# leonardsiegert/PULPo

Measured on AMD Instinct MI355X. Metric: volume-pairs/sec fwd+bwd, 160^3 fp32, higher is better.
Workload: dtype f32

## Files before the change

### include/pulpo_hip.h

```cpp
#ifndef PULPO_HIP_H
#define PULPO_HIP_H

#include <stddef.h>
#include <stdint.h>

#ifdef __cplusplus
extern "C" {
#endif

#define PULPO_ABI_VERSION 8
int pulpo_abi_version(void);
const char* pulpo_last_error(void);

size_t pulpo_conv3d_k3_packed_floats(int K, int N);
int pulpo_conv3d_k3_pack_weight(const float* w , float* wp, int Cin, int Cout, int dgrad, void* stream);
int pulpo_conv3d_k3_stat_tiles(int B, int D, int H, int W);
int pulpo_conv3d_k3_tile_config(int K, int N);
size_t pulpo_conv3d_k3_fwd_scratch_floats(int B, int D, int H, int W, int K, int N);
int pulpo_conv3d_k3_fwd(const float* in, int64_t in_bs, int64_t in_ps, int64_t in_cs, const float* wp, const float* bias, float* out,
                        int64_t out_bs, int64_t out_ps, int64_t out_cs, float* stats, float* scratch , int B,
                        int D, int H, int W, int K, int N, void* stream);
int pulpo_conv3d_k3_fwd_bn_lrelu(const float* in, int64_t in_bs, int64_t in_ps, int64_t in_cs, const float* wp, const float* bias,
                                 const float* coef, float slope, float* out, int64_t out_bs, int64_t out_ps, int64_t out_cs, float* scratch, int B,
                                 int D, int H, int W, int K, int N, void* stream);
// ... 231 lines not shown
int pulpo_bn_lrelu_apply_t(const void* y, int y_dt, int64_t yps, void* z, int z_dt, int64_t zps, const float* coef, int64_t npix, int C, float slope,
                           void* stream);
int pulpo_bn_lrelu_apply_pool2_t(const void* y, int y_dt, int64_t yps, void* z , int z_dt, int64_t zps,
                                 void* pooled , int64_t pps,
                                 const float* coef, int B, int D, int H, int W, int C, float slope, void* stream);
int pulpo_bn_lrelu_bwd_reduce_t(const void* dz, int dz_dt, int64_t dzps, const void* y, int y_dt, int64_t yps, const float* coef, int64_t npix, int C,
                                float slope, float* partial, void* stream);
int pulpo_bn_lrelu_bwd_apply_t(const void* dz, int dz_dt, int64_t dzps, const void* y, int y_dt, int64_t yps, const float* coef, const double* totd,
                               void* dy , int64_t dyps, int64_t npix, int C, float slope, float* partial2, void* stream);
int pulpo_avgpool2_bwd_bnred_t(const void* gout, int64_t gops, const void* add, int64_t aps, void* gin, int64_t gips, int g_dt ,
                               const void* y, int y_dt, int64_t yps, const float* coef, float slope, float* partial, int B, int D, int H, int W,
                               int C, void* stream);
int pulpo_heads_fwd_t(const void* h, int h_dt, int64_t ps, const float* Wt, const float* bias, const float* eps, float* o0, float* o1, float* o2,
                      int nout, int B, int64_t V, int C, void* stream);
int pulpo_heads_bwd_t(const void* h, int h_dt, int64_t ps, const float* Wt, const float* g0, const float* g1, const float* g2, const float* eps,
                      const float* sigma, void* dh , int64_t dps, float* partial, int nout, int B, int64_t V, int C, void* stream);
int pulpo_avgpool2_fwd_t(const void* in, int64_t ips, void* out, int64_t ops, int dt, int B, int D, int H, int W, int C, void* stream);
int pulpo_avgpool2_bwd_t(const void* gout, int64_t gops, const void* add , int64_t aps, void* gin, int64_t gips, int dt, int B, int D,
                         int H, int W, int C, void* stream);
int pulpo_feedback_up2_fwd_t(const float* const* srcs , const int* chans , int nsrc, void* out,
                             int dt, int64_t ops, int B, int Di, int Hi, int Wi, void* stream);
int pulpo_feedback_up2_bwd_t(const void* gout, int dt, int64_t gops, float* const* gsrcs , const int* chans,
                             int nsrc, int B, int Di, int Hi, int Wi, void* stream);

int pulpo_conv3d_k3_wgrad_bn_rows(int B, int D, int H, int W, int Cout);
int pulpo_conv3d_k3_wgrad_bn(const float* in, int64_t in_bs, int64_t in_ps, int64_t in_cs, const void* dz, int dz_dt, int64_t dz_bs, int64_t dz_ps,
                             const float* y, int64_t y_bs, int64_t y_ps, const float* coef, const double* totd, float slope, float* dw,
                             int accumulate, float* scratch, float* part2, int B, int D, int H, int W, int Cin, int Cout, void* stream);

int pulpo_bn_lrelu_bwd_apply_pooled_t(const void* gout, int64_t gops, const void* add , int64_t aps, int g_dt, const void* y, int y_dt,
                                      int64_t yps, const float* coef, const double* totd, void* dy , int64_t dyps, float slope,
                                      float* partial2, int B, int D, int H, int W, int C, void* stream);

int pulpo_bn_lrelu_apply_kb(const float* y, int64_t yps, float* z, int64_t zps, int64_t zkb, const float* coef, int64_t npix, int C, float slope, void* stream);
int pulpo_bn_lrelu_bwd_apply_kb_t(const void* dz, int dz_dt, int64_t dzps, int64_t dzkb, const float* y, int64_t yps, const float* coef, const double* totd,
                                  float* dy, int64_t dyps, int64_t dykb, int64_t npix, int C, float slope, float* partial2, void* stream);
int pulpo_conv3d_k3_wgrad_bn_kb(const float* in, int64_t in_bs, int64_t in_ps, int64_t in_cs, const float* dz, int64_t dz_bs, int64_t dz_ps, int64_t dz_kb,
                                const float* y, int64_t y_bs, int64_t y_ps, const float* coef, const double* totd, float slope, float* dw, int accumulate,
                                float* scratch, float* part2, int B, int D, int H, int W, int Cin, int Cout, void* stream);
int pulpo_bn_lrelu_bwd_apply_pooled_kb_t(const void* gout, int64_t gops, const void* add , int64_t aps, int g_dt, const float* y, int64_t yps,
                                         const float* coef, const double* totd, float* dy, int64_t dyps, int64_t dykb, float slope, float* partial2,
                                         int B, int D, int H, int W, int C, void* stream);
int pulpo_conv3d_k3_fwd_wino3_kb(const float* in, int64_t in_bs, int64_t in_ps, int64_t in_kb, const float* wp, const float* bias, const float* coef,
                                 float slope, float* out, int64_t out_bs, int64_t out_ps, int64_t out_kb, float* stats, int B, int D, int H, int W, int K,
                                 int N, void* stream);
int pulpo_conv3d_k3_dgrad_wino3_bnred_kb(const float* in, int64_t in_bs, int64_t in_ps, int64_t in_kb, const float* wp, float* out, int64_t out_bs,
                                         int64_t out_ps, int64_t out_kb, const float* bn_y, int64_t bn_y_bs, int64_t bn_y_ps, const float* bn_coef, float slope,
                                         float* part, int B, int D, int H, int W, int K, int N, void* stream);
int pulpo_conv3d_k3_wgrad_kb(const float* in, int64_t in_bs, int64_t in_ps, int64_t in_kb, const float* dy, int64_t dy_bs, int64_t dy_ps, int64_t dy_kb,
                             float* dw, int accumulate, float* scratch, float* slabs , int nslab, int B, int D, int H, int W, int Cin, int Cout,
                             void* stream);

int pulpo_conv3d_k3_wgrad_det_slabs(int Cin, int Cout);
int pulpo_conv3d_k3_wgrad_det(const float* in, int64_t in_bs, int64_t in_ps, int64_t in_cs, const float* dy, int64_t dy_bs, int64_t dy_ps,
                              int64_t dy_cs, float* dw, int accumulate, float* scratch, float* slabs, int nslab, int B, int D, int H, int W,
                              int Cin, int Cout, void* stream);
int pulpo_conv3d_k3_wgrad_bf16_det_t(const void* in, int64_t in_bs, int64_t in_ps, int64_t in_cs, const void* dy, int64_t dy_bs, int64_t dy_ps,
                                     int64_t dy_cs, int dt, float* dw, int accumulate, float* scratch, float* slabs, int nslab, int B, int D,
                                     int H, int W, int Cin, int Cout, void* stream);
int pulpo_resize_trilinear_scaled_bwd_det(const float* gout, float* gin, int64_t nplanes, int Di, int Hi, int Wi, int Do, int Ho, int Wo,
                                          float scale_d, float scale_h, float scale_w, float mult, void* stream);
size_t pulpo_warp3d_bwd_det_ws_bytes(int B, int C, int Di, int Hi, int Wi);
int pulpo_warp3d_bwd_det(const float* df, const float* img, const float* gout, float* gdf , float* gimg ,
                         void* ws , int B, int C, int Dg, int Hg, int Wg, int Di, int Hi, int Wi, void* stream);
size_t pulpo_vecint_bwd_det_ws_bytes(int B, int D, int H, int W, int nsteps);
int pulpo_vecint_bwd_det(const float* work, const float* gout, float* gin, void* ws , int B, int D, int H, int W,
// ... 30 lines not shown
```

### pulpo_amd/csrc/norm_act.hip

```cpp
#include "act_io.h"
#include "head_bn.h"

namespace {

__global__ __launch_bounds__(1024) void colsum_kernel(const float* __restrict__ partials, int nrow, int ncol, float* __restrict__ out,
                                                        float scale, int accumulate) {
    __shared__ double red[32][33];
    const int cx = threadIdx.x, ry = threadIdx.y;
    const int c = blockIdx.x * 32 + cx;
    double s = 0.0;
    if (c < ncol)
        for (int r = ry; r < nrow; r += 32) s += (double)partials[(long)r * ncol + c];
    red[ry][cx] = s;
    __syncthreads();
    if (ry == 0 && c < ncol) {
        double t = 0.0;
#pragma unroll
        for (int k = 0; k < 32; ++k) t += red[k][cx];
        const float r = (float)(t * (double)scale);
        out[c] = accumulate ? out[c] + r : r;
    }
}

constexpr int CS_RY = 8;
// ... 86 lines not shown
    coef[2 * C + c] = sc;
    coef[3 * C + c] = beta[c] - rm[c] * sc;
    double* cd = reinterpret_cast<double*>(coef + 4 * C);
    cd[c] = (double)rm[c];
    cd[C + c] = 1.0 / sqrt((double)rv[c] + (double)eps);
}

template <int VEC>
struct Vec {
    static __device__ __forceinline__ void ld(const float* p, float (&v)[VEC]) { pulpo::ldv<VEC>(p, v); }
    static __device__ __forceinline__ void st(float* p, const float (&v)[VEC]) { pulpo::stv<VEC>(p, v); }
};

template <int VEC, typename TY = float, typename TZ = float>
__global__ __launch_bounds__(256) void bn_lrelu_apply_kernel(const TY* __restrict__ y, long yps, TZ* __restrict__ z, long zps,
                                                               const float* __restrict__ coef, long npix, int C, float slope, long zkb = 8) {
    const int CV = C / VEC;
    const long total = npix * CV;
    const float* scale = coef + 2 * C;
    const float* shift = coef + 3 * C;
    for (long e = blockIdx.x * (long)blockDim.x + threadIdx.x; e < total; e += (long)gridDim.x * blockDim.x) {
        const long p = e / CV;
        const int c = (int)(e - p * CV) * VEC;
        float v[VEC], sc[VEC], sh[VEC];
        pulpo::ldv<VEC>(y + p * yps + c, v);
        Vec<VEC>::ld(scale + c, sc);
        Vec<VEC>::ld(shift + c, sh);
#pragma unroll
        for (int k = 0; k < VEC; ++k) v[k] = pulpo::bn_lrelu(v[k], sc[k], sh[k], slope);
        pulpo::stv<VEC>(z + (long)(c >> 3) * zkb + p * zps + (c & 7), v);
    }
}

template <typename TY = float, typename TZ = float>
__global__ __launch_bounds__(256) void bn_lrelu_apply_pool2_kernel(const TY* __restrict__ y, long yps, TZ* __restrict__ z, long zps,
                                                                     TZ* __restrict__ pooled, long pps, const float* __restrict__ coef, int B,
                                                                     int D, int H, int W, int Do, int Ho, int Wo, int C, float slope) {
    const int CV = C / 4;
    const long total = (long)B * Do * Ho * Wo * CV;
    const float* scale = coef + 2 * C;
    const float* shift = coef + 3 * C;
    for (long e = blockIdx.x * (long)blockDim.x + threadIdx.x; e < total; e += (long)gridDim.x * blockDim.x) {
        const int c = (int)(e % CV) * 4;
        long p = e / CV;
        const int ox = (int)(p % Wo); p /= Wo;
        const int oy = (int)(p % Ho); p /= Ho;
        const int oz = (int)(p % Do);
        const int b = (int)(p / Do);
        const int z1 = min(2 * oz + 2, D), y1 = min(2 * oy + 2, H), x1 = min(2 * ox + 2, W);
        float sc[4], sh[4], acc[4] = {0.f, 0.f, 0.f, 0.f};
        Vec<4>::ld(scale + c, sc);
        Vec<4>::ld(shift + c, sh);
        for (int zz = 2 * oz; zz < z1; ++zz)
            for (int yy = 2 * oy; yy < y1; ++yy)
                for (int xx = 2 * ox; xx < x1; ++xx) {
                    const long vox = (((long)b * D + zz) * H + yy) * W + xx;
                    float v[4];
                    pulpo::ldv<4>(y + vox * yps + c, v);
#pragma unroll
                    for (int k = 0; k < 4; ++k) {
                        v[k] = pulpo::as_stored<TZ>(pulpo::bn_lrelu(v[k], sc[k], sh[k], slope));
                        acc[k] += v[k];
                    }
                    if (z != nullptr) pulpo::stv<4>(z + vox * zps + c, v);
                }
        const float inv = 1.f / (float)((z1 - 2 * oz) * (y1 - 2 * oy) * (x1 - 2 * ox));
#pragma unroll
        for (int k = 0; k < 4; ++k) acc[k] *= inv;
        pulpo::stv<4>(pooled + ((((long)b * Do + oz) * Ho + oy) * Wo + ox) * pps + c, acc);
    }
}

template <typename TG>
struct PoolGrad {
    const TG* gpool; long gpps;
    const TG* add; long aps;
    TG* dzout; long dzops;
    int D, H, W, Do, Ho, Wo;
};

template <int VEC, bool POOL = false, typename TG = float, typename TY = float>
__global__ __launch_bounds__(256) void bn_lrelu_bwd_reduce_kernel(const TG* __restrict__ dz, long dzps, const TY* __restrict__ y,
                                                                    long yps, const float* __restrict__ coef, long npix, int C,
                                                                    float slope, float* __restrict__ partial, PoolGrad<TG> pg = PoolGrad<TG>{}) {
    extern __shared__ float red[];
    const int CV = C / VEC, RB = blockDim.x / CV;
    const int col = threadIdx.x % CV, row = threadIdx.x / CV;
    const int c = col * VEC;
    float s0[VEC], s1[VEC];
#pragma unroll
    for (int k = 0; k < VEC; ++k) s0[k] = s1[k] = 0.f;
    if (row < RB) {
        float sc[VEC], sh[VEC], m32[VEC];
        Vec<VEC>::ld(coef + 2 * C + c, sc);
        Vec<VEC>::ld(coef + 3 * C + c, sh);
        Vec<VEC>::ld(coef + c, m32);
        for (long p = (long)blockIdx.x * RB + row; p < npix; p += (long)gridDim.x * RB) {
            float g[VEC], v[VEC];
            if constexpr (POOL) {
                long q = p;
                const int x_ = (int)(q % pg.W); q /= pg.W;
                const int y_ = (int)(q % pg.H); q /= pg.H;
// ... 244 lines not shown
                                   void* stream) {
    return pulpo_bn_lrelu_apply_t(y, 0, yps, z, 0, zps, coef, npix, C, slope, stream);
}

PULPO_API int pulpo_bn_lrelu_apply_kb(const float* y, int64_t yps, float* z, int64_t zps, int64_t zkb, const float* coef, int64_t npix, int C, float slope,
                                      void* stream) {
    PULPO_REQUIRE(y && z && coef && npix > 0 && C > 0 && C % 8 == 0 && zps % 4 == 0 && zps >= 8 && zkb % 4 == 0 && zkb >= 8, "bn_lrelu_apply_kb: bad arguments");
    return apply_t(y, (long)yps, z, (long)zps, coef, (long)npix, C, slope, (hipStream_t)stream, (long)zkb);
}

PULPO_API int pulpo_bn_lrelu_apply_pool2_ok(int C, int64_t yps, int64_t zps, int64_t pps) { return C % 4 == 0 && yps % 4 == 0 && zps % 4 == 0 && pps % 4 == 0; }

PULPO_API int pulpo_bn_lrelu_apply_pool2_t(const void* y, int y_dt, int64_t yps, void* z, int z_dt, int64_t zps, void* pooled, int64_t pps,
                                           const float* coef, int B, int D, int H, int W, int C, float slope, void* stream) {
    PULPO_REQUIRE(y && pooled && coef && B > 0 && D > 0 && H > 0 && W > 0 && C > 0, "bn_lrelu_apply_pool2: bad arguments");
    PULPO_REQUIRE_DT(y_dt, "bn_lrelu_apply_pool2"); PULPO_REQUIRE_DT(z_dt, "bn_lrelu_apply_pool2");
    const int ey = y_dt ? 2 : 4, ez = z_dt ? 2 : 4;
    PULPO_REQUIRE(pulpo_bn_lrelu_apply_pool2_ok(C, yps, zps, pps) && (((uintptr_t)y) % (4 * ey)) == 0 && ((((uintptr_t)z) | ((uintptr_t)pooled)) % (4 * ez)) == 0 &&
                      (((uintptr_t)coef) & 15) == 0,
                  "bn_lrelu_apply_pool2: operands must be channels-last, aligned to four elements, C %% 4 == 0");
    const int Do = (D + 1) / 2, Ho = (H + 1) / 2, Wo = (W + 1) / 2;
    const int nb = stream_blocks((long)B * Do * Ho * Wo * (C / 4));
    PULPO_DISPATCH_DT(y_dt, TY, PULPO_DISPATCH_DT(z_dt, TZ,
        hipLaunchKernelGGL((bn_lrelu_apply_pool2_kernel<TY, TZ>), dim3(nb), dim3(256), 0, (hipStream_t)stream, (const TY*)y, (long)yps, (TZ*)z, (long)zps,
                           (TZ*)pooled, (long)pps, coef, B, D, H, W, Do, Ho, Wo, C, slope)));
    return pulpo::check_launch("bn_lrelu_apply_pool2");
}

PULPO_API int pulpo_bn_lrelu_apply_pool2(const float* y, int64_t yps, float* z, int64_t zps, float* pooled, int64_t pps, const float* coef, int B, int D,
                                         int H, int W, int C, float slope, void* stream) {
    return pulpo_bn_lrelu_apply_pool2_t(y, 0, yps, z, 0, zps, pooled, pps, coef, B, D, H, W, C, slope, stream);
}

PULPO_API int pulpo_bn_bwd_blocks(int64_t npix, int C) {
    const int vec = (C % 4 == 0) ? 4 : 1;
    const int RB = std::max(1, 256 / (C / vec));
    return (int)std::max<long>(1, std::min<long>((npix + RB * 8 - 1) / (RB * 8), 2048));
}

namespace {
inline int bwd_group(const pulpo::GroupProbe& g, bool half, int C) {
    if (half && g.ok8 && C / 8 <= 256) return 8;
    if (g.ok4) return C / 4 <= 256 ? 4 : -2;
    if (C % 4 == 0) return -1;
    return C <= 256 ? 1 : -2;
}

template <typename TG, typename TY>
int reduce_t(const TG* dz, long dzps, const TY* y, long yps, const float* coef, long npix, int C, float slope, float* partial, hipStream_t st) {
    pulpo::GroupProbe g(C);
    g.add(dz, dzps, sizeof(TG)); g.add(y, yps, sizeof(TY)); g.add(coef, 8, 4);
    const int vec = bwd_group(g, sizeof(TG) == 2 || sizeof(TY) == 2, C);
    if (vec == -1) return pulpo::fail(-1, "bn_lrelu_bwd_reduce: operands must be aligned to four elements when C %% 4 == 0");
    if (vec == -2) return pulpo::fail(-1, "bn_lrelu_bwd_reduce: too many channels (%d)", C);
    const int nblk = pulpo_bn_bwd_blocks(npix, C);
    const int RB = std::max(1, 256 / (C / vec));
    const size_t lds = (size_t)RB * 2 * C * sizeof(float);
    if (vec == 8) hipLaunchKernelGGL((bn_lrelu_bwd_reduce_kernel<8, false, TG, TY>), dim3(nblk), dim3(256), lds, st, dz, dzps, y, yps, coef, npix, C, slope, partial, PoolGrad<TG>{});
    else if (vec == 4) hipLaunchKernelGGL((bn_lrelu_bwd_reduce_kernel<4, false, TG, TY>), dim3(nblk), dim3(256), lds, st, dz, dzps, y, yps, coef, npix, C, slope, partial, PoolGrad<TG>{});
    else hipLaunchKernelGGL((bn_lrelu_bwd_reduce_kernel<1, false, TG, TY>), dim3(nblk), dim3(256), lds, st, dz, dzps, y, yps, coef, npix, C, slope, partial, PoolGrad<TG>{});
    return pulpo::check_launch("bn_lrelu_bwd_reduce");
}

template <typename TG, typename TY>
int pool_reduce_t(const TG* gout, long gops, const TG* add, long aps, TG* gin, long gips, const TY* y, long yps, const float* coef, float slope,
                  float* partial, int B, int D, int H, int W, int C, hipStream_t st) {
// ... 41 lines not shown
                                          int C, float slope, float* partial, void* stream) {
    PULPO_REQUIRE(dz && y && coef && partial && npix > 0 && C > 0, "bn_lrelu_bwd_reduce: bad arguments");
    PULPO_REQUIRE_DT(dz_dt, "bn_lrelu_bwd_reduce"); PULPO_REQUIRE_DT(y_dt, "bn_lrelu_bwd_reduce");
    PULPO_DISPATCH_DT(dz_dt, TG, PULPO_DISPATCH_DT(y_dt, TY,
        return reduce_t((const TG*)dz, (long)dzps, (const TY*)y, (long)yps, coef, (long)npix, C, slope, partial, (hipStream_t)stream)));
    return -1;
}

PULPO_API int pulpo_bn_lrelu_bwd_reduce(const float* dz, int64_t dzps, const float* y, int64_t yps, const float* coef, int64_t npix, int C,
                                        float slope, float* partial, void* stream) {
    return pulpo_bn_lrelu_bwd_reduce_t(dz, 0, dzps, y, 0, yps, coef, npix, C, slope, partial, stream);
}

PULPO_API int pulpo_avgpool2_bwd_bnred_t(const void* gout, int64_t gops, const void* add, int64_t aps, void* gin, int64_t gips, int g_dt, const void* y,
                                         int y_dt, int64_t yps, const float* coef, float slope, float* partial, int B, int D, int H, int W, int C,
                                         void* stream) {
    PULPO_REQUIRE(gout && y && coef && partial && B > 0 && D > 0 && H > 0 && W > 0 && C > 0, "avgpool2_bwd_bnred: bad arguments");
    PULPO_REQUIRE_DT(g_dt, "avgpool2_bwd_bnred"); PULPO_REQUIRE_DT(y_dt, "avgpool2_bwd_bnred");
    const int eg = g_dt ? 8 : 16, ey = y_dt ? 8 : 16;
    PULPO_REQUIRE(C % 4 == 0 && C / 4 <= 256 && gops % 4 == 0 && gips % 4 == 0 && yps % 4 == 0 && (add == nullptr || aps % 4 == 0) &&
                      ((((uintptr_t)gout) | ((uintptr_t)gin) | ((uintptr_t)add)) % eg) == 0 && (((uintptr_t)y) % ey) == 0 && (((uintptr_t)coef) & 15) == 0,
                  "avgpool2_bwd_bnred: operands must be channels-last, aligned to four elements, C %% 4 == 0");
    PULPO_DISPATCH_DT(g_dt, TG, PULPO_DISPATCH_DT(y_dt, TY,
        return pool_reduce_t((const TG*)gout, (long)gops, (const TG*)add, (long)aps, (TG*)gin, (long)gips, (const TY*)y, (long)yps, coef, slope, partial, B, D,
                             H, W, C, (hipStream_t)stream)));
    return -1;
}

PULPO_API int pulpo_avgpool2_bwd_bnred(const float* gout, int64_t gops, const float* add, int64_t aps, float* gin, int64_t gips, const float* y,
                                       int64_t yps, const float* coef, float slope, float* partial, int B, int D, int H, int W, int C, void* stream) {
    return pulpo_avgpool2_bwd_bnred_t(gout, gops, add, aps, gin, gips, 0, y, 0, yps, coef, slope, partial, B, D, H, W, C, stream);
}

PULPO_API int pulpo_bn_lrelu_bwd_apply_pooled_t(const void* gout, int64_t gops, const void* add, int64_t aps, int g_dt, const void* y, int y_dt, int64_t yps,
                                                const float* coef, const double* totd, void* dy, int64_t dyps, float slope, float* partial2, int B, int D,
                                                int H, int W, int C, void* stream) {
    PULPO_REQUIRE(gout && y && coef && totd && dy && partial2 && B > 0 && D > 0 && H > 0 && W > 0 && C > 0, "bn_lrelu_bwd_apply_pooled: bad arguments");
    PULPO_REQUIRE_DT(g_dt, "bn_lrelu_bwd_apply_pooled"); PULPO_REQUIRE_DT(y_dt, "bn_lrelu_bwd_apply_pooled");
    const int eg = g_dt ? 8 : 16, ey = y_dt ? 8 : 16;
    PULPO_REQUIRE(C % 4 == 0 && C / 4 <= 256 && gops % 4 == 0 && yps % 4 == 0 && dyps % 4 == 0 && (add == nullptr || aps % 4 == 0) &&
                      ((((uintptr_t)gout) | ((uintptr_t)add)) % eg) == 0 && ((((uintptr_t)y) | ((uintptr_t)dy)) % ey) == 0 && (((uintptr_t)coef) & 15) == 0,
                  "bn_lrelu_bwd_apply_pooled: operands must be channels-last, aligned to four elements, C %% 4 == 0");
    PULPO_DISPATCH_DT(g_dt, TG, PULPO_DISPATCH_DT(y_dt, TY,
        return pool_apply_t((const TG*)gout, (long)gops, (const TG*)add, (long)aps, (const TY*)y, (long)yps, coef, totd, (TY*)dy, (long)dyps, slope, partial2, B,
                            D, H, W, C, (hipStream_t)stream)));
    return -1;
}

PULPO_API size_t pulpo_bn_bwd_finalize_scratch_doubles(int ntile, int C) { return ntile > 2048 ? (size_t)32 * 2 * C : 0; }

PULPO_API int pulpo_bn_bwd_finalize(const float* tile_part, int ntile, int C, const float* coef, double count, int use_means, float* dbeta,
                                          float* dgamma, int accumulate, double* totd, double* scratch, void* stream) {
    PULPO_REQUIRE(tile_part && coef && dbeta && dgamma && totd && ntile > 0 && C > 0 && count > 0, "bn_bwd_finalize: bad arguments");
    hipStream_t st = (hipStream_t)stream;
    const double* partd = nullptr;
    int nrow = ntile;
    if (pulpo_bn_bwd_finalize_scratch_doubles(ntile, C) != 0) {
        PULPO_REQUIRE(scratch != nullptr, "bn_bwd_finalize: scratch required for %d tiles", ntile);
        hipLaunchKernelGGL(colsum_slices_kernel, dim3(pulpo::cdiv(2 * C, 32), 32), dim3(32, CS_RY), 0, st, tile_part, ntile, 2 * C, scratch);
        int rc = pulpo::check_launch("bn backward tile slices");
        if (rc) return rc;
        partd = scratch;
        nrow = 32;
    }
    hipLaunchKernelGGL(bn_bwd_finalize_kernel, dim3(pulpo::cdiv(C, 8)), dim3(8, 64), 0, st, tile_part, partd, nrow, C, coef, count, use_means,
                       dbeta, dgamma, accumulate, totd);
// ... 46 lines not shown
```

### pulpo_amd/dp.py

```python
from __future__ import annotations

import os
from typing import Iterable, List, Optional

import torch
import torch.distributed as dist
import torch.nn as nn


class FlatArena:

    ALIGN = 4

    def __init__(self, module: nn.Module, params: Optional[List[nn.Parameter]] = None):
        self.module_order: List[nn.Parameter] = [p for p in module.parameters() if p.requires_grad]
        self.module_names: List[str] = [n for n, p in module.named_parameters() if p.requires_grad]
        if params is None:
            params = list(self.module_order)
        elif {id(p) for p in params} != {id(p) for p in module.parameters() if p.requires_grad}:
            raise ValueError("FlatArena: `params` must be a permutation of the module's trainable parameters")
        if not params:
            raise ValueError("FlatArena: module has no trainable parameters")
        dev, dt = params[0].device, params[0].dtype
        self.params: List[nn.Parameter] = params
# ... 318 lines not shown
                    levels = getattr(model, "_pulpo_last_reg_levels", None)
            finally:
                model._pulpo_in_graph = False
            self._graph = (g, static, loss.detach(), levels, self._signature(batch))
            self.reduce_and_update()
            return loss_w
        g, static, loss, levels, _ = self._graph
        for dst, src in zip(static, batch):
            if dst.numel() and dst.data_ptr() != src.data_ptr():
                dst.copy_(src, non_blocking=True)
        if hasattr(model, "_check_previous_step_for_nan"):
            model._check_previous_step_for_nan()
        g.replay()
        if levels is not None and hasattr(model, "_arm_nan_probe"):
            model._arm_nan_probe(levels)
        self.reduce_and_update()
        return loss

    def wgrad_on_side_stream(self) -> bool:
        if not self.async_wgrad:
            return False
        force = os.environ.get("PULPO_WGRAD_SIDE_STREAM", "auto")
        if force in ("0", "1"):
            return force == "1"
        from . import ops
        return ops.CONV_PRECISION == "bf16"

    def coarse_window(self) -> bool:
        from . import ops
        return bool(self._want_window and self._window is not None and not self.wgrad_on_side_stream() and not ops.DETERMINISTIC
                    and ops.CONV_PRECISION == "fp32")

    def describe(self) -> dict:
        w = self._window
        return {"overlap": bool(self.overlap and world() > 1), "async_wgrad": bool(self.async_wgrad), "wgrad_side_stream": self.wgrad_on_side_stream(),
                "buckets": len(self.buckets), "coarse_window": self.coarse_window(),
                "coarse_window_settings": None if w is None else {"coarse_voxels": w.coarse_voxels, "max_workgroups": w.max_workgroups,
                                                                  "defer_flop": w.defer_flop, "exit_wait": w.exit_wait, "deferred_last_step": w.deferred_last}}


class ArenaAdam(torch.optim.Adam):

    def __init__(self, model: nn.Module, lr: float = 1e-4, **stepper_kw):
        super().__init__([p for p in model.parameters() if p.requires_grad], lr=lr)
        self.engine = DataParallelStepper(model, lr=lr, **stepper_kw)
        self.reduced_elsewhere = False

    def zero_grad(self, set_to_none: bool = True) -> None:
        self.engine.zero_grad()

    @torch.no_grad()
    def step(self, closure=None):
        loss = None
        if closure is not None:
            with torch.enable_grad():
                loss = closure()
        g = self.param_groups[0]
        fa = self.engine.opt
        fa.lr, fa.betas, fa.eps = float(g["lr"]), tuple(g["betas"]), float(g["eps"])
        if g.get("weight_decay", 0) or g.get("amsgrad") or g.get("maximize"):
            raise ValueError("ArenaAdam: weight_decay / amsgrad / maximize are not part of the reference's optimizer (models.py:399)")
        self.engine.reduce_and_update(reduced_elsewhere=self.reduced_elsewhere)
        return loss

    def state_dict(self) -> dict:
        sd = self.engine.opt.state_dict()
        sd["param_groups"][0].update({k: v for k, v in self.param_groups[0].items() if k not in ("params",) and k in sd["param_groups"][0]})
        return sd

# ... 19 lines not shown
```

### pulpo_amd/ops.py

```python
from __future__ import annotations

import collections
import contextlib
import ctypes
import os
from typing import Optional, Sequence, Tuple

import torch

from ._lib import PulpoHipError, lib

CL = torch.channels_last_3d
LRELU_SLOPE = 0.2


def _ptr(t: Optional[torch.Tensor]):
    return None if t is None else ctypes.c_void_p(t.data_ptr())


def _stream():
    return ctypes.c_void_p(torch.cuda.current_stream().cuda_stream)


def _require_gpu(*ts: Optional[torch.Tensor], act: bool = False):
# ... 185 lines not shown


CONV_PRECISION = "fp32"
ACT_BF16 = False
CONV_ALGO = None


def set_conv_precision(precision: str, activations: str = "fp32") -> None:
    global CONV_PRECISION, ACT_BF16
    if precision not in ("fp32", "bf16"):
        raise ValueError(f"conv precision is {precision}. Not a known option.")
    if activations not in ("fp32", "bf16") or (activations == "bf16" and precision != "bf16"):
        raise ValueError(f"activation storage is {activations} with {precision} operands. Not a known option.")
    CONV_PRECISION = precision
    ACT_BF16 = activations == "bf16"


def act_dtype():
    return torch.bfloat16 if ACT_BF16 else torch.float32


DETERMINISTIC = os.environ.get("PULPO_DETERMINISTIC", "0") == "1"


def set_deterministic(on: bool = True) -> None:
    global DETERMINISTIC
    DETERMINISTIC = bool(on)


BN_REDUCE_IN_DGRAD = True
FUSE_INPUT_WGRAD = True
POOLED_BN_BACKWARD = True
FUSE_HEAD_BN = True


def _use_bf16(K: int) -> bool:
    return CONV_PRECISION == "bf16" and K > 4


_WEIGHT_EPOCH = 0


def invalidate_weight_packs() -> None:
    global _WEIGHT_EPOCH
    _WEIGHT_EPOCH += 1
    _PACK_REGISTRY.clear()


_PACK_REGISTRY: dict = {}
_PACK_TABLES: dict = {}
_UNREFRESHABLE_PACKS = False
_registrations = 0


def _register_pack(w: torch.Tensor, wp: torch.Tensor, Cin: int, Cout: int, dgrad: bool, kind: int) -> None:
    global _registrations
    import weakref
    _PACK_REGISTRY[id(wp)] = (weakref.ref(w), wp, Cin, Cout, dgrad, kind)
    _registrations += 1
    if _registrations % 64 == 0:
        for k in [k for k, e in _PACK_REGISTRY.items() if e[0]() is None]:
            del _PACK_REGISTRY[k]


def refresh_weight_packs() -> None:
    global _UNREFRESHABLE_PACKS
# ... 531 lines not shown
    def forward(ctx, a, b, buf):
        ctx.ca = a.shape[1]
        return buf.as_strided(buf.shape, buf.stride(), buf.storage_offset())

    @staticmethod
    def backward(ctx, g):
        return g[:, :ctx.ca], g[:, ctx.ca:], None


def cat_channels(a: torch.Tensor, b: torch.Tensor) -> torch.Tensor:
    ta, tb = getattr(a, "_pulpo_cat", None), getattr(b, "_pulpo_cat", None)
    if ta is not None and tb is not None and ta[0] is tb[0]:
        buf = ta[0]
        es = buf.element_size()
        if (ta[1] == 0 and tb[1] == a.shape[1] and a.shape[1] + b.shape[1] == buf.shape[1] and a.data_ptr() == buf.data_ptr()
                and b.data_ptr() == buf.data_ptr() + es * tb[1] and a.stride() == buf.stride() and b.stride() == buf.stride()
                and a.shape[2:] == buf.shape[2:] and b.shape[2:] == buf.shape[2:] and a.shape[0] == buf.shape[0] == b.shape[0]):
            global CAT_PREWRITTEN_HITS
            CAT_PREWRITTEN_HITS += 1
            return _CatPrewritten.apply(a, b, buf)
    return torch.cat([a, b], dim=1)


class _UnitCall:
    __slots__ = ("bn_src", "out", "pool_after", "pool_only", "blocked_out", "training", "momentum", "eps", "running_mean", "running_var",
                 "num_batches_tracked", "head_nout", "head_eps", "head_params", "y", "coef", "pooled", "pool_only_done")

    def __init__(self, **given):
        assert not set(given) - set(self.__slots__), given
        for name in self.__slots__:
            setattr(self, name, given.get(name))


_DzSource = collections.namedtuple("_DzSource", "dz blk pooled head", defaults=(None, False, None, None))


def _unit_grads(dx=None, dw=None, dbias=None, dgamma=None, dbeta=None, head_dw=None, head_db=None):
    return dx, dw, dbias, dgamma, dbeta, head_dw, head_db, None


def _fwd_heads(y, coef, head_w, head_b, head_eps, nout: int, dims):
    _require_gpu(head_w, head_b, head_eps)
    B, Cout, D, H, W = dims
    V = D * H * W
    outs = [torch.empty((B, 3, D, H, W), device=y.device, dtype=torch.float32) for _ in range(1 if nout == 3 else 3)]
    epsc = planar(head_eps) if head_eps is not None else None
    t0 = _hbm_begin("heads_fwd_bn")
    lib.call("pulpo_heads_fwd_bn_t", _ptr(y), y.stride(4), _ptr(coef), LRELU_SLOPE, _ptr(head_w), _ptr(head_b), _ptr(epsc), _ptr(outs[0]),
             _ptr(outs[1]) if nout == 6 else None, _ptr(outs[2]) if nout == 6 else None, nout, B, V, Cout, _stream())
    _hbm_end(t0, "heads_fwd_bn", B * V * (4.0 * Cout + 4.0 * (12 if nout == 6 else 3)))
    return outs, epsc


def _fwd_bn_lrelu_apply(y, coef, call, dims, zdt):
    B, Cout, D, H, W = dims
    dev, npix = y.device, B * D * H * W
    pool_only = bool(call.pool_only and call.pool_after and lib.query("pulpo_bn_lrelu_apply_pool2_ok", Cout, y.stride(4), Cout, Cout))
    blocked_out = bool(call.blocked_out and call.training and not call.pool_after and not pool_only and zdt == y.dtype == torch.float32 and Cout % 8 == 0)
    z = None if (pool_only or blocked_out) else _out_slot(call.out, B, Cout, D, H, W, dev, zdt)
    if z is None and not pool_only and not blocked_out:
        z = new_cl(B, Cout, D, H, W, dev, zdt)
    pooled = None
    if blocked_out:
        global BLOCKED_Z_HITS
        BLOCKED_Z_HITS += 1
        z = torch.empty((Cout // 8, B, D, H, W, 8), device=dev, dtype=torch.float32)
        entry, args = "pulpo_bn_lrelu_apply_kb", (_ptr(y), y.stride(4), _ptr(z), 8, npix * 8, _ptr(coef), npix, Cout, LRELU_SLOPE)
    elif pool_only or (call.pool_after and lib.query("pulpo_bn_lrelu_apply_pool2_ok", Cout, y.stride(4), z.stride(4), Cout)):
        pooled = new_cl(B, Cout, (D + 1) // 2, (H + 1) // 2, (W + 1) // 2, dev, zdt)
        entry, args = "pulpo_bn_lrelu_apply_pool2_t", (_ptr(y), _dt(y), y.stride(4), _ptr(z), _dt(pooled), z.stride(4) if z is not None else Cout, _ptr(pooled),
                                                       pooled.stride(4), _ptr(coef), B, D, H, W, Cout, LRELU_SLOPE)
    else:
        entry, args = "pulpo_bn_lrelu_apply_t", (_ptr(y), _dt(y), y.stride(4), _ptr(z), _dt(z), z.stride(4), _ptr(coef), npix, Cout, LRELU_SLOPE)
    t0 = _hbm_begin("bn_lrelu_apply")
    lib.call(entry, *args, _stream())
    _hbm_end(t0, "bn_lrelu_apply", (_esize(y) + (0 if pool_only else (2.0 if zdt == torch.bfloat16 else 4.0))) * Cout * npix)
    return z, pooled, pool_only


class _ConvBNLReLU(torch.autograd.Function):

    @staticmethod
    def forward(ctx, x, weight, bias, gamma, beta, head_w, head_b, call: _UnitCall):
        _require_gpu(x, act=True)
        _require_gpu(weight, bias, gamma, beta)
        training = call.training
        ctx.bn_src = call.bn_src
        ctx.dx_blocked = is_blocked(x)
        if not ctx.dx_blocked:
            x = as_grid(x)
        B, Cin, D, H, W = _dims5(x)
        Cout = weight.shape[0]
        dev = x.device
        wp = _pack_weight(weight, dgrad=False, shape=(B, D, H, W), both=bool(training and ctx.needs_input_grad[0]))
        half_conv = ACT_BF16 and wp._pulpo_algo == "bf16"
        if ctx.dx_blocked and (wp._pulpo_algo != "wino3" or half_conv or not training):
            x = blocked_to_cl(x)
        if x.dtype != (torch.bfloat16 if half_conv else torch.float32):
            x = x.to(torch.bfloat16 if half_conv else torch.float32)
        ydt = torch.bfloat16 if half_conv else torch.float32
        zdt = act_dtype()
        y = new_cl(B, Cout, D, H, W, dev, ydt)
        coef = torch.empty(8 * Cout, device=dev, dtype=torch.float32)
        if training:
            ntile = lib.query("pulpo_conv3d_k3_fwd_bf16_stat_tiles" if wp._pulpo_algo == "bf16" else "pulpo_conv3d_k3_stat_tiles", B, D, H, W)
            stats = torch.empty(ntile * 2 * Cout, device=dev, dtype=torch.float32)
            _conv_raw(x, wp, bias, y, Cin, Cout, stats)
            nsd = lib.query("pulpo_bn_fwd_finalize_scratch_doubles", ntile, Cout)
            scratch = torch.empty(nsd, device=dev, dtype=torch.float64) if nsd else None
            lib.call("pulpo_bn_fwd_finalize", _ptr(stats), ntile, Cout, float(B * D * H * W), _ptr(gamma), _ptr(beta), _ptr(call.running_mean),
                     _ptr(call.running_var), _ptr(call.num_batches_tracked), call.momentum, call.eps, _ptr(coef), _ptr(scratch), _stream())
        else:
            lib.call("pulpo_bn_eval_coef", _ptr(gamma), _ptr(beta), _ptr(call.running_mean), _ptr(call.running_var), call.eps, Cout, _ptr(coef), _stream())
            if not any(ctx.needs_input_grad) and ydt == zdt:
                zo = _out_slot(call.out, B, Cout, D, H, W, dev, zdt)
                if zo is not None:
                    y = zo
                _conv_raw(x, wp, bias, y, Cin, Cout, None, coef=coef)
                return y
            _conv_raw(x, wp, bias, y, Cin, Cout, None)
        ctx.training = training
        ctx.params = (weight, bias, gamma, beta)
        ctx.pool_only = False
        ctx.head = (call.head_nout, call.head_params) if call.head_nout else None
        if call.head_nout:
            outs, epsc = _fwd_heads(y, coef, head_w, head_b, call.head_eps, call.head_nout, (B, Cout, D, H, W))
            ctx.save_for_backward(x, weight, y, coef, head_w, epsc, outs[1] if call.head_nout == 6 else None)
            return outs[0] if call.head_nout == 3 else tuple(outs)
        z, pooled, pool_only = _fwd_bn_lrelu_apply(y, coef, call, (B, Cout, D, H, W), zdt)
        ctx.save_for_backward(x, weight, y, coef)
        call.y, call.coef, call.pooled, call.pool_only_done = y, coef, pooled, pool_only
        ctx.pool_only = pool_only
        if pool_only:
            ctx.set_materialize_grads(False)
            return pooled
        if pooled is not None:
            ctx.set_materialize_grads(False)
            return z, pooled
        return z

    @staticmethod
    def backward(ctx, *grads):
        x, weight, y, coef = ctx.saved_tensors[:4]
        need_dx, need_dw, need_db = ctx.needs_input_grad[:3]
        B, Cin, D, H, W = _dims5(x)
        dims = (B, Cin, weight.shape[0], D, H, W)
        nblk = lib.query("pulpo_bn_bwd_blocks", B * D * H * W, dims[2])
        src = _bwd_dz_source(grads, ctx.head, ctx.pool_only, ctx.saved_tensors, y, dims)
        if src is None:
            return _unit_grads()
        src, totd, slot_w, slot_b, dgamma, dbeta, head_dw, head_db = _bwd_bn_sums(
            src, y, coef, dims, nblk, ctx.training, ctx.params, ctx.needs_input_grad, ctx.head)
        wpt = _pack_weight(weight, dgrad=True, shape=(B, D, H, W)) if need_dx else None
        dy, bias_rows = _bwd_bn_apply(src, x, weight, y, coef, totd, wpt, dims, nblk, (need_dx, need_dw, need_db), ctx.params[1], slot_b)
        dw, dbias, side_job = _bwd_param_grads(src, x, dy, bias_rows, y, coef, totd, dims, (need_dw, need_db), ctx.params, slot_w, slot_b)
        dx = _bwd_data_grad(x, dy, wpt, ctx.bn_src, ctx.dx_blocked, dims, side_job)
        return _unit_grads(dx, dw, dbias, dgamma, dbeta, head_dw, head_db)


def _bwd_dz_source(grads, head, pool_only: bool, saved, y, dims) -> Optional[_DzSource]:
    B, _, Cout, D, H, W = dims
    dev = y.device
    dz, dpool, dsample = (grads + (None, None))[:3]
    if head is not None:
        g = [planar(t) if t is not None else None for t in (dz, dpool, dsample)]
        if head[0] == 3 and g[0] is None:
            g[0] = torch.zeros((B, 3, D, H, W), device=dev)
        hw, heps, hsigma = saved[4:7]
        return _DzSource(head=(head[0], (_ptr(hw), _ptr(g[0]), _ptr(g[1]), _ptr(g[2]), _ptr(heps), _ptr(hsigma)), (hw, g, heps, hsigma)))
    if pool_only:
        dz, dpool = None, dz
    dz_blk = is_blocked(dz)
    if dz_blk and (dz.dtype != torch.float32 or not dz.is_contiguous() or tuple(blocked_shape(dz)) != (B, Cout, D, H, W)):
        dz, dz_blk = blocked_to_cl(dz.float()), False
    if dpool is None:
        if dz is None:
            return None
        return _DzSource(dz if dz_blk else to_cl(dz), dz_blk)
    gp = to_cl(dpool)
    gz = dz
    if gz is not None and gz.dtype != gp.dtype:
        gz = gz.to(gp.dtype)
    grp = 4 * int(_esize(gp))
    skip_ok = gz is None
    if gz is not None:
        sb, sp, _ = grid_strides(gz)
        skip_ok = _dense_grid(gz) and sb == D * H * W * sp and _vec4(gz, align=grp, batch=False)
    if (Cout // 4 <= 256 and skip_ok and _vec4(gp, Cout, align=grp, batch=False) and _vec4(y, align=4 * int(_esize(y)), batch=False)
            and _dense_grid(y) and POOLED_BN_BACKWARD):
        return _DzSource(pooled=(gp, gz))
    gin = new_cl(B, Cout, D, H, W, dev, gp.dtype)
    add = skip_ok and gz is not None
    lib.call("pulpo_avgpool2_bwd_t", _ptr(gp), gp.stride(4), _ptr(gz) if add else None, grid_strides(gz)[1] if add else 0, _ptr(gin), gin.stride(4), _dt(gp),
             B, D, H, W, Cout, _stream())
    return _DzSource(to_cl(gin if (add or gz is None) else gin + gz), False)


def _bwd_bn_sums(src: _DzSource, y, coef, dims, nblk: int, training: bool, params, needs, head):
    B, _, Cout, D, H, W = dims
    dev, npix = y.device, B * D * H * W
    head_dw = head_db = None
    if src.pooled is not None:
        gp, gz = src.pooled
        rows, nrow = torch.empty(nblk * 2 * Cout, device=dev, dtype=torch.float32), nblk
        t0 = _hbm_begin("avgpool2_bwd_bnred")
        lib.call("pulpo_avgpool2_bwd_bnred_t", _ptr(gp), gp.stride(4), _ptr(gz), grid_strides(gz)[1] if gz is not None else 0, None, 0, _dt(gp), _ptr(y), _dt(y),
                 y.stride(4), _ptr(coef), LRELU_SLOPE, _ptr(rows), B, D, H, W, Cout, _stream())
        _hbm_end(t0, "avgpool2_bwd_bnred", Cout * (_esize(gp) * (gp.numel() // Cout + (npix if gz is not None else 0)) + _esize(y) * npix))
    elif src.head is not None:
        (nout, hparams), V = head, D * H * W
        nrow = lib.query("pulpo_heads_bwd_blocks", B, V, Cout)
        hpart, hslots = _heads_part_rows(hparams, needs[5] and needs[6], nrow, nout, Cout, dev)
        rows = torch.empty(nrow * 2 * Cout, device=dev, dtype=torch.float32)
        t0 = _hbm_begin("heads_bwd_bn")
        lib.call("pulpo_heads_bwd_bn_t", _ptr(y), y.stride(4), _ptr(coef), LRELU_SLOPE, *src.head[1], _ptr(hpart), _ptr(rows), nout, B, V, Cout, _stream())
        _hbm_end(t0, "heads_bwd_bn", B * V * (4.0 * Cout + 4.0 * (15 if nout == 6 else 3)))
        head_dw, head_db = _heads_finish_rows(hpart, hslots, hparams, nrow, nout, Cout)
    else:
        tiles = _take_bn_tile_parts(y, coef, src.dz)
        if tiles is not None:
            rows, nrow = tiles
        else:
            if src.blk:
                src = _DzSource(blocked_to_cl(src.dz), False)
            dz = src.dz
            rows, nrow = torch.empty(nblk * 2 * Cout, device=dev, dtype=torch.float32), nblk
            t0 = _hbm_begin("bn_lrelu_bwd_reduce")
            lib.call("pulpo_bn_lrelu_bwd_reduce_t", _ptr(dz), _dt(dz), dz.stride(4), _ptr(y), _dt(y), y.stride(4), _ptr(coef), npix, Cout, LRELU_SLOPE,
                     _ptr(rows), _stream())
            _hbm_end(t0, "bn_lrelu_bwd_reduce", (_esize(dz) + _esize(y)) * Cout * npix)
    if _PASS.window is not None:
        _PASS.window.visit(D * H * W)
    slot_w, slot_b, slot_g, slot_be = (_grad_slot(t) if need else None for t, need in zip(params, needs[1:5]))
    direct_bn = slot_g is not None and slot_be is not None
    tot = None if direct_bn else torch.empty(2 * Cout, device=dev, dtype=torch.float32)
# ... 1874 lines not shown
```

Before: 39.65.

## Precompute pooled BN-backward sums in forward pool kernel to skip full-res reread

The forward BN+LReLU+avgpool kernel now also emits, per pooled voxel, two per-channel partial sums: the count of LReLU slopes and the slope-weighted centered activation. A new backward reduction kernel combines these with the pooled gradient, so the BN-backward channel sums no longer reread the full-resolution activation. This replaces a full-res read in backward with two extra pooled-size writes in forward and reads in backward. It applies only to fp32, pool-only layers without a skip gradient, and volumes at or above a size threshold.

Result: no change. 39.69, median of 3 (+0.1%).

```diff
diff --git a/include/pulpo_hip.h b/include/pulpo_hip.h
--- a/include/pulpo_hip.h
+++ b/include/pulpo_hip.h
@@ -287,6 +287,13 @@
                                       int64_t yps, const float* coef, const double* totd, void* dy , int64_t dyps, float slope,
                                       float* partial2, int B, int D, int H, int W, int C, void* stream);
 
+int pulpo_bn_lrelu_apply_pool2_sums_ok(int C, int64_t yps, int64_t zps, int64_t pps, int64_t sps);
+int pulpo_bn_lrelu_apply_pool2_sums_t(const void* y, int y_dt, int64_t yps, void* z , int z_dt, int64_t zps, void* pooled , int64_t pps,
+                                      float* s0, float* s1, int64_t sps, const float* coef, int B, int D, int H, int W, int C, float slope, void* stream);
+int pulpo_avgpool2_bwd_bnred_sums_rows(int B, int D, int H, int W, int C);
+int pulpo_avgpool2_bwd_bnred_sums(const float* gout, int64_t gops, const float* s0, const float* s1, int64_t sps, float* partial, int B, int D, int H, int W,
+                                  int C, void* stream);
+
 int pulpo_bn_lrelu_apply_kb(const float* y, int64_t yps, float* z, int64_t zps, int64_t zkb, const float* coef, int64_t npix, int C, float slope, void* stream);
 int pulpo_bn_lrelu_bwd_apply_kb_t(const void* dz, int dz_dt, int64_t dzps, int64_t dzkb, const float* y, int64_t yps, const float* coef, const double* totd,
                                   float* dy, int64_t dyps, int64_t dykb, int64_t npix, int C, float slope, float* partial2, void* stream);
diff --git a/pulpo_amd/csrc/norm_act.hip b/pulpo_amd/csrc/norm_act.hip
--- a/pulpo_amd/csrc/norm_act.hip
+++ b/pulpo_amd/csrc/norm_act.hip
@@ -142,10 +142,10 @@
     }
 }
 
-template <typename TY = float, typename TZ = float>
-__global__ __launch_bounds__(256) void bn_lrelu_apply_pool2_kernel(const TY* __restrict__ y, long yps, TZ* __restrict__ z, long zps,
-                                                                     TZ* __restrict__ pooled, long pps, const float* __restrict__ coef, int B,
-                                                                     int D, int H, int W, int Do, int Ho, int Wo, int C, float slope) {
+template <bool SUMS, typename TY, typename TZ>
+__device__ __forceinline__ void apply_pool2_body(const TY* __restrict__ y, long yps, TZ* __restrict__ z, long zps, TZ* __restrict__ pooled, long pps,
+                                                 float* __restrict__ s0out, float* __restrict__ s1out, long sps, const float* __restrict__ coef, int B,
+                                                 int D, int H, int W, int Do, int Ho, int Wo, int C, float slope) {
     const int CV = C / 4;
     const long total = (long)B * Do * Ho * Wo * CV;
     const float* scale = coef + 2 * C;
@@ -161,6 +161,8 @@
         float sc[4], sh[4], acc[4] = {0.f, 0.f, 0.f, 0.f};
         Vec<4>::ld(scale + c, sc);
         Vec<4>::ld(shift + c, sh);
+        float m32[4], t0[4] = {0.f, 0.f, 0.f, 0.f}, t1[4] = {0.f, 0.f, 0.f, 0.f};
+        if constexpr (SUMS) Vec<4>::ld(coef + c, m32);
         for (int zz = 2 * oz; zz < z1; ++zz)
             for (int yy = 2 * oy; yy < y1; ++yy)
                 for (int xx = 2 * ox; xx < x1; ++xx) {
@@ -169,6 +171,12 @@
                     pulpo::ldv<4>(y + vox * yps + c, v);
 #pragma unroll
                     for (int k = 0; k < 4; ++k) {
+                        if constexpr (SUMS) {
+                            const float bn = v[k] * sc[k] + sh[k];
+                            const float l = bn > 0.f ? 1.f : slope;
+                            t0[k] += l;
+                            t1[k] = fmaf(l, v[k] - m32[k], t1[k]);
+                        }
                         v[k] = pulpo::as_stored<TZ>(pulpo::bn_lrelu(v[k], sc[k], sh[k], slope));
                         acc[k] += v[k];
                     }
@@ -177,7 +185,68 @@
         const float inv = 1.f / (float)((z1 - 2 * oz) * (y1 - 2 * oy) * (x1 - 2 * ox));
 #pragma unroll
         for (int k = 0; k < 4; ++k) acc[k] *= inv;
-        pulpo::stv<4>(pooled + ((((long)b * Do + oz) * Ho + oy) * Wo + ox) * pps + c, acc);
+        const long po = (((long)b * Do + oz) * Ho + oy) * Wo + ox;
+        pulpo::stv<4>(pooled + po * pps + c, acc);
+        if constexpr (SUMS) {
+            Vec<4>::st(s0out + po * sps + c, t0);
+            Vec<4>::st(s1out + po * sps + c, t1);
+        }
+    }
+}
+
+template <typename TY = float, typename TZ = float>
+__global__ __launch_bounds__(256) void bn_lrelu_apply_pool2_kernel(const TY* __restrict__ y, long yps, TZ* __restrict__ z, long zps,
+                                                                     TZ* __restrict__ pooled, long pps, const float* __restrict__ coef, int B,
+                                                                     int D, int H, int W, int Do, int Ho, int Wo, int C, float slope) {
+    apply_pool2_body<false>(y, yps, z, zps, pooled, pps, (float*)nullptr, (float*)nullptr, 0L, coef, B, D, H, W, Do, Ho, Wo, C, slope);
+}
+
+template <typename TY = float, typename TZ = float>
+__global__ __launch_bounds__(256) void bn_lrelu_apply_pool2_sums_kernel(const TY* __restrict__ y, long yps, TZ* __restrict__ z, long zps,
+                                                                          TZ* __restrict__ pooled, long pps, float* __restrict__ s0out,
+                                                                          float* __restrict__ s1out, long sps, const float* __restrict__ coef, int B,
+                                                                          int D, int H, int W, int Do, int Ho, int Wo, int C, float slope) {
+    apply_pool2_body<true>(y, yps, z, zps, pooled, pps, s0out, s1out, sps, coef, B, D, H, W, Do, Ho, Wo, C, slope);
+}
+
+__global__ __launch_bounds__(256) void pool_sums_bwd_reduce_kernel(const float* __restrict__ gpool, long gpps, const float* __restrict__ s0in,
+                                                                     const float* __restrict__ s1in, long sps, long npp, int D, int H, int W, int Do,
+                                                                     int Ho, int Wo, int C, float* __restrict__ partial) {
+    extern __shared__ float red[];
+    const int CV = C / 4, RB = blockDim.x / CV;
+    const int col = threadIdx.x % CV, row = threadIdx.x / CV;
+    const int c = col * 4;
+    float a0[4] = {0.f, 0.f, 0.f, 0.f}, a1[4] = {0.f, 0.f, 0.f, 0.f};
+    if (row < RB) {
+        for (long p = (long)blockIdx.x * RB + row; p < npp; p += (long)gridDim.x * RB) {
+            long q = p;
+            const int ox = (int)(q % Wo); q /= Wo;
+            const int oy = (int)(q % Ho); q /= Ho;
+            const int oz = (int)(q % Do);
+            const int cnt = (min(2 * oz + 2, D) - 2 * oz) * (min(2 * oy + 2, H) - 2 * oy) * (min(2 * ox + 2, W) - 2 * ox);
+            const float inv = 1.f / (float)cnt;
+            float g[4], u0[4], u1[4];
+            pulpo::ldv<4>(gpool + p * gpps + c, g);
+            Vec<4>::ld(s0in + p * sps + c, u0);
+            Vec<4>::ld(s1in + p * sps + c, u1);
+#pragma unroll
+            for (int k = 0; k < 4; ++k) {
+                const float gk = g[k] * inv;
+                a0[k] = fmaf(gk, u0[k], a0[k]);
+                a1[k] = fmaf(gk, u1[k], a1[k]);
+            }
+        }
+#pragma unroll
+        for (int k = 0; k < 4; ++k) {
+            red[(row * 2 + 0) * C + c + k] = a0[k];
+            red[(row * 2 + 1) * C + c + k] = a1[k];
+        }
+    }
+    __syncthreads();
+    for (int j = threadIdx.x; j < 2 * C; j += blockDim.x) {
+        float t = 0.f;
+        for (int r = 0; r < RB; ++r) t += red[r * 2 * C + j];
+        partial[(long)blockIdx.x * 2 * C + j] = t;
     }
 }
 
@@ -488,6 +557,26 @@
     return pulpo_bn_lrelu_apply_pool2_t(y, 0, yps, z, 0, zps, pooled, pps, coef, B, D, H, W, C, slope, stream);
 }
 
+PULPO_API int pulpo_bn_lrelu_apply_pool2_sums_ok(int C, int64_t yps, int64_t zps, int64_t pps, int64_t sps) {
+    return pulpo_bn_lrelu_apply_pool2_ok(C, yps, zps, pps) && sps % 4 == 0 && sps >= C && C / 4 <= 256;
+}
+
+PULPO_API int pulpo_bn_lrelu_apply_pool2_sums_t(const void* y, int y_dt, int64_t yps, void* z, int z_dt, int64_t zps, void* pooled, int64_t pps, float* s0,
+                                                float* s1, int64_t sps, const float* coef, int B, int D, int H, int W, int C, float slope, void* stream) {
+    PULPO_REQUIRE(y && pooled && s0 && s1 && coef && B > 0 && D > 0 && H > 0 && W > 0 && C > 0, "bn_lrelu_apply_pool2_sums: bad arguments");
+    PULPO_REQUIRE_DT(y_dt, "bn_lrelu_apply_pool2_sums"); PULPO_REQUIRE_DT(z_dt, "bn_lrelu_apply_pool2_sums");
+    const int ey = y_dt ? 2 : 4, ez = z_dt ? 2 : 4;
+    PULPO_REQUIRE(pulpo_bn_lrelu_apply_pool2_sums_ok(C, yps, zps, pps, sps) && (((uintptr_t)y) % (4 * ey)) == 0 &&
+                      ((((uintptr_t)z) | ((uintptr_t)pooled)) % (4 * ez)) == 0 && ((((uintptr_t)coef) | ((uintptr_t)s0) | ((uintptr_t)s1)) & 15) == 0,
+                  "bn_lrelu_apply_pool2_sums: operands must be channels-last, aligned to four elements, C %% 4 == 0");
+    const int Do = (D + 1) / 2, Ho = (H + 1) / 2, Wo = (W + 1) / 2;
+    const int nb = stream_blocks((long)B * Do * Ho * Wo * (C / 4));
+    PULPO_DISPATCH_DT(y_dt, TY, PULPO_DISPATCH_DT(z_dt, TZ,
+        hipLaunchKernelGGL((bn_lrelu_apply_pool2_sums_kernel<TY, TZ>), dim3(nb), dim3(256), 0, (hipStream_t)stream, (const TY*)y, (long)yps, (TZ*)z, (long)zps,
+                           (TZ*)pooled, (long)pps, s0, s1, (long)sps, coef, B, D, H, W, Do, Ho, Wo, C, slope)));
+    return pulpo::check_launch("bn_lrelu_apply_pool2_sums");
+}
+
 PULPO_API int pulpo_bn_bwd_blocks(int64_t npix, int C) {
     const int vec = (C % 4 == 0) ? 4 : 1;
     const int RB = std::max(1, 256 / (C / vec));
@@ -595,6 +684,26 @@
     return pulpo_avgpool2_bwd_bnred_t(gout, gops, add, aps, gin, gips, 0, y, 0, yps, coef, slope, partial, B, D, H, W, C, stream);
 }
 
+PULPO_API int pulpo_avgpool2_bwd_bnred_sums_rows(int B, int D, int H, int W, int C) {
+    return pulpo_bn_bwd_blocks((int64_t)B * ((D + 1) / 2) * ((H + 1) / 2) * ((W + 1) / 2), C);
+}
+
+PULPO_API int pulpo_avgpool2_bwd_bnred_sums(const float* gout, int64_t gops, const float* s0, const float* s1, int64_t sps, float* partial, int B, int D, int H,
+                                            int W, int C, void* stream) {
+    PULPO_REQUIRE(gout && s0 && s1 && partial && B > 0 && D > 0 && H > 0 && W > 0 && C > 0, "avgpool2_bwd_bnred_sums: bad arguments");
+    PULPO_REQUIRE(C % 4 == 0 && C / 4 <= 256 && gops % 4 == 0 && gops >= C && sps % 4 == 0 && sps >= C &&
+                      ((((uintptr_t)gout) | ((uintptr_t)s0) | ((uintptr_t)s1)) & 15) == 0,
+                  "avgpool2_bwd_bnred_sums: operands must be fp32, channels-last, aligned to four elements, C %% 4 == 0");
+    const int Do = (D + 1) / 2, Ho = (H + 1) / 2, Wo = (W + 1) / 2;
+    const long npp = (long)B * Do * Ho * Wo;
+    const int nblk = pulpo_avgpool2_bwd_bnred_sums_rows(B, D, H, W, C);
+    const int RB = std::max(1, 256 / (C / 4));
+    const size_t lds = (size_t)RB * 2 * C * sizeof(float);
+    hipLaunchKernelGGL(pool_sums_bwd_reduce_kernel, dim3(nblk), dim3(256), lds, (hipStream_t)stream, gout, (long)gops, s0, s1, (long)sps, npp, D, H, W, Do, Ho,
+                       Wo, C, partial);
+    return pulpo::check_launch("avgpool2_bwd_bnred_sums");
+}
+
 PULPO_API int pulpo_bn_lrelu_bwd_apply_pooled_t(const void* gout, int64_t gops, const void* add, int64_t aps, int g_dt, const void* y, int y_dt, int64_t yps,
                                                 const float* coef, const double* totd, void* dy, int64_t dyps, float slope, float* partial2, int B, int D,
                                                 int H, int W, int C, void* stream) {
diff --git a/pulpo_amd/dp.py b/pulpo_amd/dp.py
--- a/pulpo_amd/dp.py
+++ b/pulpo_amd/dp.py
@@ -374,9 +374,11 @@
                     and ops.CONV_PRECISION == "fp32")
 
     def describe(self) -> dict:
+        from . import ops
         w = self._window
         return {"overlap": bool(self.overlap and world() > 1), "async_wgrad": bool(self.async_wgrad), "wgrad_side_stream": self.wgrad_on_side_stream(),
                 "buckets": len(self.buckets), "coarse_window": self.coarse_window(),
+                "pooled_bn_sums": {"on": bool(ops.POOLED_BN_SUMS), "min_voxels": int(ops.POOLED_BN_SUMS_MIN_VOXELS)},
                 "coarse_window_settings": None if w is None else {"coarse_voxels": w.coarse_voxels, "max_workgroups": w.max_workgroups,
                                                                   "defer_flop": w.defer_flop, "exit_wait": w.exit_wait, "deferred_last_step": w.deferred_last}}
 
diff --git a/pulpo_amd/ops.py b/pulpo_amd/ops.py
--- a/pulpo_amd/ops.py
+++ b/pulpo_amd/ops.py
@@ -241,6 +241,9 @@
 FUSE_INPUT_WGRAD = True
 POOLED_BN_BACKWARD = True
 FUSE_HEAD_BN = True
+POOLED_BN_SUMS = True
+POOLED_BN_SUMS_MIN_VOXELS = 96 ** 3
+POOLED_BN_SUMS_HITS = 0
 
 
 def _use_bf16(K: int) -> bool:
@@ -838,7 +841,7 @@
             setattr(self, name, given.get(name))
 
 
-_DzSource = collections.namedtuple("_DzSource", "dz blk pooled head", defaults=(None, False, None, None))
+_DzSource = collections.namedtuple("_DzSource", "dz blk pooled head sums", defaults=(None, False, None, None, None))
 
 
 def _unit_grads(dx=None, dw=None, dbias=None, dgamma=None, dbeta=None, head_dw=None, head_db=None):
@@ -858,7 +861,7 @@
     return outs, epsc
 
 
-def _fwd_bn_lrelu_apply(y, coef, call, dims, zdt):
+def _fwd_bn_lrelu_apply(y, coef, call, dims, zdt, want_sums: bool = False):
     B, Cout, D, H, W = dims
     dev, npix = y.device, B * D * H * W
     pool_only = bool(call.pool_only and call.pool_after and lib.query("pulpo_bn_lrelu_apply_pool2_ok", Cout, y.stride(4), Cout, Cout))
@@ -866,7 +869,7 @@
     z = None if (pool_only or blocked_out) else _out_slot(call.out, B, Cout, D, H, W, dev, zdt)
     if z is None and not pool_only and not blocked_out:
         z = new_cl(B, Cout, D, H, W, dev, zdt)
-    pooled = None
+    pooled = sums = None
     if blocked_out:
         global BLOCKED_Z_HITS
         BLOCKED_Z_HITS += 1
@@ -876,12 +879,17 @@
         pooled = new_cl(B, Cout, (D + 1) // 2, (H + 1) // 2, (W + 1) // 2, dev, zdt)
         entry, args = "pulpo_bn_lrelu_apply_pool2_t", (_ptr(y), _dt(y), y.stride(4), _ptr(z), _dt(pooled), z.stride(4) if z is not None else Cout, _ptr(pooled),
                                                        pooled.stride(4), _ptr(coef), B, D, H, W, Cout, LRELU_SLOPE)
+        if (pool_only and want_sums and POOLED_BN_SUMS and D * H * W >= POOLED_BN_SUMS_MIN_VOXELS and zdt == y.dtype == torch.float32
+                and lib.query("pulpo_bn_lrelu_apply_pool2_sums_ok", Cout, y.stride(4), Cout, Cout, Cout)):
+            sums = torch.empty((2,) + tuple(pooled.shape[:1] + pooled.shape[2:]) + (Cout,), device=dev, dtype=torch.float32)
+            entry, args = "pulpo_bn_lrelu_apply_pool2_sums_t", args[:8] + (_ptr(sums[0]), _ptr(sums[1]), Cout) + args[8:]
     else:
         entry, args = "pulpo_bn_lrelu_apply_t", (_ptr(y), _dt(y), y.stride(4), _ptr(z), _dt(z), z.stride(4), _ptr(coef), npix, Cout, LRELU_SLOPE)
     t0 = _hbm_begin("bn_lrelu_apply")
     lib.call(entry, *args, _stream())
-    _hbm_end(t0, "bn_lrelu_apply", (_esize(y) + (0 if pool_only else (2.0 if zdt == torch.bfloat16 else 4.0))) * Cout * npix)
-    return z, pooled, pool_only
+    _hbm_end(t0, "bn_lrelu_apply", (_esize(y) + (0 if pool_only else (2.0 if zdt == torch.bfloat16 else 4.0))) * Cout * npix
+             + (4.0 * sums.numel() if sums is not None else 0.0))
+    return z, pooled, pool_only, sums
 
 
 class _ConvBNLReLU(torch.autograd.Function):
@@ -933,8 +941,8 @@
             outs, epsc = _fwd_heads(y, coef, head_w, head_b, call.head_eps, call.head_nout, (B, Cout, D, H, W))
             ctx.save_for_backward(x, weight, y, coef, head_w, epsc, outs[1] if call.head_nout == 6 else None)
             return outs[0] if call.head_nout == 3 else tuple(outs)
-        z, pooled, pool_only = _fwd_bn_lrelu_apply(y, coef, call, (B, Cout, D, H, W), zdt)
-        ctx.save_for_backward(x, weight, y, coef)
+        z, pooled, pool_only, sums = _fwd_bn_lrelu_apply(y, coef, call, (B, Cout, D, H, W), zdt, want_sums=bool(training and any(ctx.needs_input_grad[:5])))
+        ctx.save_for_backward(x, weight, y, coef, sums)
         call.y, call.coef, call.pooled, call.pool_only_done = y, coef, pooled, pool_only
         ctx.pool_only = pool_only
         if pool_only:
@@ -953,6 +961,8 @@
         dims = (B, Cin, weight.shape[0], D, H, W)
         nblk = lib.query("pulpo_bn_bwd_blocks", B * D * H * W, dims[2])
         src = _bwd_dz_source(grads, ctx.head, ctx.pool_only, ctx.saved_tensors, y, dims)
+        if src is not None and src.pooled is not None and src.pooled[1] is None and ctx.head is None and ctx.saved_tensors[4] is not None:
+            src = src._replace(sums=ctx.saved_tensors[4])
         if src is None:
             return _unit_grads()
         src, totd, slot_w, slot_b, dgamma, dbeta, head_dw, head_db = _bwd_bn_sums(
@@ -1006,7 +1016,16 @@
     B, _, Cout, D, H, W = dims
     dev, npix = y.device, B * D * H * W
     head_dw = head_db = None
-    if src.pooled is not None:
+    if src.pooled is not None and src.sums is not None and src.pooled[0].dtype == torch.float32:
+        global POOLED_BN_SUMS_HITS
+        POOLED_BN_SUMS_HITS += 1
+        gp, sums = src.pooled[0], src.sums
+        nrow = lib.query("pulpo_avgpool2_bwd_bnred_sums_rows", B, D, H, W, Cout)
+        rows = torch.empty(nrow * 2 * Cout, device=dev, dtype=torch.float32)
+        t0 = _hbm_begin("avgpool2_bwd_bnred_sums")
+        lib.call("pulpo_avgpool2_bwd_bnred_sums", _ptr(gp), gp.stride(4), _ptr(sums[0]), _ptr(sums[1]), Cout, _ptr(rows), B, D, H, W, Cout, _stream())
+        _hbm_end(t0, "avgpool2_bwd_bnred_sums", 4.0 * 3 * (gp.numel() // Cout) * Cout)
+    elif src.pooled is not None:
         gp, gz = src.pooled
         rows, nrow = torch.empty(nblk * 2 * Cout, device=dev, dtype=torch.float32), nblk
         t0 = _hbm_begin("avgpool2_bwd_bnred")
```
